# thnak/image_super_resolution

Measured on AMD Instinct MI355X. Metric: 4x SR megapixels/sec (HR output) + PSNR vs reference CPU path, higher is better.
Workload: dtype fp16; 1 GPU; ResNet(16, 0.2, scaleRate=4) RRDB inference, 128x128->512x512; global_batch=16, per_gpu_batch=16, lr_size=128, scale=4, parallelism=dp1 (independent tile shards), streams_per_gpu=1, hip_graph=True, trunk=persistent chain kernel, storage=fp16 activations and packed weights, fp32 accumulation

## Files before the change

### image_super_resolution_amd/csrc/trunk.hip

```cpp
#include "trunk_common.h"

namespace isr {

size_t trunk_state_words(int n, int ha, int wa) {
    const size_t tiles = (size_t)n * (ha / tk::TH) * (wa / tk::TW);
    return trunk_rec_off((int)tiles) + 1024 * 16;
}

__global__ __launch_bounds__(1024) void trunk_prep_kernel(const isr_conv_desc* layers, const int32_t* kinds, int nl,
                                                          int n, int ha, int wa, unsigned* state, int th,
                                                          int h16) {
    extern __shared__ __attribute__((aligned(16))) char smem[];
    unsigned* err = reinterpret_cast<unsigned*>(smem);
    const int L = threadIdx.x;
    const int nbx = wa / tk::TW, nby = ha / th, ntiles = n * nbx * nby;
    const size_t ro = trunk_rec_off(ntiles);
    if (L == 0) *err = 0;
    __syncthreads();
    const isr_conv_desc& g0 = layers[0];
    if (L < nl) {
        const isr_conv_desc& d = layers[L];
        unsigned e = 0;
        auto same_geo = [&](const isr_view& v) {
            return v.hp == g0.x.hp && v.wp == g0.x.wp && v.cs == g0.x.cs && v.pad == g0.x.pad && v.coff % 16 == 0 &&
                   v.pad >= 1;
        };
        const int kind = kinds[L];
        const bool masked = kind == 2;
        if (d.n != n || d.ha != ha || d.wa != wa || d.h != g0.h || d.w != g0.w) e |= 1;
        if (!same_geo(d.x) || !same_geo(d.y) || (d.r2.data && !same_geo(d.r2)) || (masked && !same_geo(d.m))) e |= 2;
        if (kind == 0 || kind == 2 ? d.cout != 32 : (kind == 1 ? d.cout != 64 : true)) e |= 4;
        if (d.cin % 16 || d.cin < 64 || d.cin / 16 > 120 || !d.bias || ((uintptr_t)d.bias & 15)) e |= 8;
        if (d.f16 != h16 || d.shuffle != 1 || d.x_sub2 || d.taps || d.y2.data || (d.m.data != nullptr) != masked ||
            (masked && (d.m_c0 != 0 || d.slope != 1.f || d.r1.data || d.r2.data || d.s1 != 1.f || d.s2 != 1.f)))
            e |= 16;
        int fold = 0;
        uint16_t idv = 0;
        if (d.r1.data) {
            const float inv = 1.f / d.s1;
            float back;
            if (h16) {
                const _Float16 hi = (_Float16)inv;
                idv = __builtin_bit_cast(uint16_t, hi);
                back = (float)hi;
            } else {
                const __bf16 bi = (__bf16)inv;
                idv = __builtin_bit_cast(uint16_t, bi);
                back = (float)bi;
            }
            const bool alias = d.r1.data == d.x.data && d.r1.coff == d.x.coff && d.r1_cn == 0;
            if (!alias || kind != 1 || d.slope != 1.f || back != inv) e |= 32;
            fold = 1;
        } else if (d.r2.data) {
            e |= 32;
        }
        int first_new = tk::NEED_NONE;
        if (L > 0) {
            const isr_conv_desc& p = layers[L - 1];
            const int lo = p.y.coff, hi = p.y.coff + p.cout;
            first_new = d.cin / 16;
            if (p.y.data == d.x.data) {
                for (int c = 0; c < d.cin / 16; ++c) {
                    const int c0 = d.x.coff + 16 * c;
                    if (c0 < hi && lo < c0 + 16) {
                        first_new = c;
                        break;
                    }
                }
            }
        }
        TrunkRec rec;
        rec.x = (uint64_t)(uintptr_t)d.x.data;
        rec.y = (uint64_t)(uintptr_t)d.y.data;
        rec.w = (uint64_t)(uintptr_t)d.wpack;
        rec.b = (uint64_t)(uintptr_t)d.bias;
        rec.r2 = (uint64_t)(uintptr_t)(masked ? d.m.data : d.r2.data);
        rec.planes = (uint32_t)(d.x.coff / 16) | (uint32_t)(d.y.coff / 16) << 16;
        rec.shape = (uint32_t)((masked ? d.m.coff : d.r2.coff) / 16) | (uint32_t)(d.cin / 16) << 16 |
                    (uint32_t)(kind & 255) << 24;
        rec.deps = (uint32_t)first_new | (uint32_t)fold << 8 | (uint32_t)idv << 16;
        rec.slope = masked ? d.mslope : d.slope;
        rec.s1 = d.s1;
        rec.s2 = d.s2;
        const uint32_t* src = reinterpret_cast<const uint32_t*>(&rec);
        uint32_t* dst = state + ro + (size_t)L * 16;
#pragma unroll
        for (int i = 0; i < 16; ++i) dst[i] = src[i];
        if (e) atomicOr(err, e);
    }
    __syncthreads();
    if (L == 0) {
        const size_t plane = (size_t)g0.x.hp * g0.x.wp * 32;
        const unsigned e = *err | (plane >= 0x7fffffffull ? 64u : 0u) | (nl > 1024 ? 128u : 0u);
        uint32_t* geo = state + ro - 16;
        const int32_t gv[16] = {n, g0.h, g0.w, ha, wa, g0.x.hp, g0.x.wp, g0.x.cs / 16, g0.x.pad, nbx, nby, ntiles,
                                (int32_t)e, 0, 0, 0};
#pragma unroll
        for (int i = 0; i < 16; ++i) geo[i] = (uint32_t)gv[i];
        state[0] = state[0] + 1u;
    }
}

int trunk_prep_launch(const isr_chain_desc* cd, int th, hipStream_t s) {
    hipLaunchKernelGGL(trunk_prep_kernel, dim3(1), dim3(1024), 16, s, cd->layers, cd->kinds, cd->nl, cd->n, cd->ha,
                       cd->wa, cd->state, th, cd->f16 ? 1 : 0);
    return hipGetLastError() == hipSuccess ? 0 : -1;
}

#ifdef ISR_TUNING
__device__ unsigned long long* g_trunk_stamps;
#endif
__device__ __forceinline__ void trunk_stamp(int L, int t, int ntiles, int slot) {
#ifdef ISR_TUNING
    unsigned long long* p = g_trunk_stamps;
    if (p != nullptr && threadIdx.x == 0 && L >= 75 && L < 90) {
        unsigned long long v;
        asm volatile("s_memrealtime %0\n\ts_waitcnt lgkmcnt(0)" : "=s"(v)::"memory");
        p[((size_t)(L - 75) * ntiles + t) * 8 + slot] = v;
    }
#else
    (void)L, (void)t, (void)ntiles, (void)slot;
#endif
}

#if ISR_TRUNK_MFMA16_PROBE
__device__ __forceinline__ f32x16 mfma32_probe16(bf16x8 a, bf16x8 b, f32x16 acc) {
    f32x4 c0 = __builtin_shufflevector(acc, acc, 0, 1, 2, 3), c1 = __builtin_shufflevector(acc, acc, 4, 5, 6, 7);
    c0 = __builtin_amdgcn_mfma_f32_16x16x32_bf16(a, b, c0, 0, 0, 0);
    c1 = __builtin_amdgcn_mfma_f32_16x16x32_bf16(a, b, c1, 0, 0, 0);
    f32x4 c2 = __builtin_shufflevector(acc, acc, 8, 9, 10, 11), c3 = __builtin_shufflevector(acc, acc, 12, 13, 14, 15);
    f32x8 lo = __builtin_shufflevector(c0, c1, 0, 1, 2, 3, 4, 5, 6, 7), hi = __builtin_shufflevector(c2, c3, 0, 1, 2, 3, 4, 5, 6, 7);
    return __builtin_shufflevector(lo, hi, 0, 1, 2, 3, 4, 5, 6, 7, 8, 9, 10, 11, 12, 13, 14, 15);
}
#endif

#ifdef ISR_TUNING
__device__ int g_trunk_knobs[4];
static int g_trunk_per_cu = 0;
__device__ __forceinline__ int trunk_abl_load() { return __builtin_amdgcn_readfirstlane(g_trunk_knobs[0]); }
#else
__device__ __forceinline__ int trunk_abl_load() { return 0; }
#endif

#ifdef ISR_TUNING
__device__ unsigned long long* g_item_stamps;
#endif
__device__ __forceinline__ void item_stamp(int L, int first_tile, int ch, int slot, int wm) {
#ifdef ISR_TUNING
    unsigned long long* p = g_item_stamps;
    const int w = wave_id();
    if (p != nullptr && first_tile && (threadIdx.x & 63) == 0 && (w == 0 || w == wm / 2) && (L == 77 || L == 79)) {
        const unsigned long long v = __builtin_amdgcn_s_memtime();
        p[((((size_t)blockIdx.x * 2 + (L == 79)) * 16 + ch) * 2 + (w != 0)) * 8 + slot] = v;
    }
#else
    (void)L, (void)first_tile, (void)ch, (void)slot, (void)wm;
#endif
}

struct TrunkArgs {
    unsigned* state;
    int rec_off;
    int nl;
    int acquire;
};


__device__ __forceinline__ void glds4(const void* gsrc, void* lds) {
    __builtin_amdgcn_global_load_lds(gsrc, ISR_LDS_PTR(lds), 4, 0, 0);
}

template <int WM_, int R_, int NST_, int TH_ = 16, int XM_ = 0, int NTP_ = 0>
struct TK {
    static constexpr int WM = WM_, R = R_, NST = NST_;
    static constexpr int HALO_AUX = 16 | ((NTP_ & 1) ? 2 : 0), STORE_AUX = 16 | ((NTP_ & 2) ? 2 : 0);
    static constexpr int XM = XM_;
    static constexpr int NT = 64 * WM;
    static constexpr int TH = TH_;
    static constexpr int HQ = (TH + 2) * tk::HC;
    static constexpr int HP = (HQ + 31) / 32;
    static_assert(R * WM == TH, "the waves cover the tile rows");
    static_assert(NST >= 2 && NST <= 4, "ring depth");
    static constexpr int HPW = (HP + WM - 1) / WM;
    static constexpr int WPW = (tk::WPF + WM - 1) / WM;
    static constexpr int SLOT = (HP + tk::WPF) * 1024;
    static constexpr int BIAS_OFF = NST * SLOT;
    static constexpr int LDS = BIAS_OFF + 4 * 256;
    static_assert(LDS <= 163840, "LDS budget");
    static constexpr int BPC = 163840 / LDS < 2 ? 163840 / LDS : 2;
    static constexpr int WPS = BPC * WM / 4;
    static constexpr int NSET = WPS >= 4 ? 1 : 2;
};

struct Src {
    const char* x;
    uint32_t h0;
    const char* w;
    const float* b;
    int wpc;
    uint32_t xbytes, wbytes;
};

template <class K>
struct TrunkCtx {
    static constexpr int TH = K::TH;
    unsigned* state;
    unsigned gen;
    int acquire;
    int hp, wp, cs16, pad, h, w, nbx, nby, ntiles;
    uint32_t pstride;
    uint32_t hoff[K::HPW];
    int abl;
};

template <class C>
__device__ __forceinline__ Src src_of(const C& c, const_rec& rec, int t) {
    const int bx = t % c.nbx, tmp = t / c.nbx, by = tmp % c.nby, img = tmp / c.nby;
    Src s;
    s.x = (const char*)(uintptr_t)rec.x + (size_t)((uint32_t)img * c.cs16 + rec_xp(rec)) * c.pstride;
    s.h0 = (uint32_t)(((by * C::TH - 1 + c.pad) * c.wp + (bx * tk::TW - 1 + c.pad)) * 32);
    s.w = (const char*)(uintptr_t)rec.w;
    s.b = (const float*)(uintptr_t)rec.b;
    s.wpc = rec_kind(rec) == 1 ? tk::WPF : tk::WPG;
    s.xbytes = c.pstride;
    s.wbytes = (uint32_t)(rec_nch(rec) * s.wpc * 1024);
    return s;
}

template <int WM, int HPW, int WPW, int SLOTB, int BIASB, int HP, int HAUX = 16>
__device__ __forceinline__ uint32_t stage_chunk_k(const uint32_t* hoff, uint32_t pstride, int abl, const Src& s,
                                                  int chunk, int slot, bool with_bias, int bslot) {
    extern __shared__ __attribute__((aligned(16))) char smem[];
    const int wave = wave_id(), lane = threadIdx.x & 63;
    char* dst = smem + slot * SLOTB;
    uint32_t n = 0;
    const auto rx = rsrc_n(s.x + (size_t)chunk * pstride, s.xbytes);
    const uint32_t so = s.h0;
    if (!(abl & 1)) {
#pragma unroll
        for (int k = 0; k < HPW; ++k) {
            const int j = wave + WM * k;
            if (j < HP) {
                __builtin_amdgcn_raw_ptr_buffer_load_lds(rx, ISR_LDS_PTR(dst + j * 1024), 16, hoff[k], so, 0, HAUX);
                ++n;
            }
        }
    }
    const auto rw = rsrc_n(s.w, s.wbytes);
    const uint32_t wo = (uint32_t)(chunk * s.wpc * 1024);
    char* wd = dst + HP * 1024;
#pragma unroll
    for (int k = 0; k < WPW; ++k) {
        const int j = wave + WM * k;
        if (j < s.wpc && !(abl & 8)) {
            __builtin_amdgcn_raw_ptr_buffer_load_lds(rw, ISR_LDS_PTR(wd + j * 1024), 16, lane * 16, wo + j * 1024, 0, 0);
            ++n;
        }
    }
    if (with_bias && wave == 0) {
        if (lane < (s.wpc == tk::WPG ? 32 : 64))
            __builtin_amdgcn_raw_ptr_buffer_load_lds(rsrc_n(s.b, s.wpc == tk::WPG ? 128u : 256u), ISR_LDS_PTR(smem + BIASB + bslot * 256), 4,
                                                     lane * 4, 0, 0, 0);
        ++n;
    }
    return n;
}

template <class K>
__device__ __forceinline__ uint32_t stage_chunk(const TrunkCtx<K>& c, const Src& s, int chunk, int slot, bool with_bias,
                                                int bslot) {
#ifdef ISR_TUNING
    if (chunk < 0 || (uint32_t)(chunk * s.wpc * 1024) >= s.wbytes || slot < 0 || slot >= K::NST ||
        bslot < 0 || bslot > 3) {
        if (threadIdx.x == 0) {
            __hip_atomic_store(c.state + 1, c.gen, __ATOMIC_RELAXED, __HIP_MEMORY_SCOPE_AGENT);
            __hip_atomic_fetch_add(c.state + 2, 1u, __ATOMIC_RELAXED, __HIP_MEMORY_SCOPE_AGENT);
        }
        return 0;
    }
#endif
    if constexpr (K::NSET == 1) {
        int ln = threadIdx.x & 63;
        asm volatile("" : "+v"(ln));
        uint32_t ho[K::HPW];
#pragma unroll
        for (int k = 0; k < K::HPW; ++k) ho[k] = halo_piece_off<K::HQ>(wave_id() + K::WM * k, ln, c.wp);
        return stage_chunk_k<K::WM, K::HPW, K::WPW, K::SLOT, K::BIAS_OFF, K::HP, K::HALO_AUX>(ho, c.pstride, c.abl, s, chunk, slot,
                                                                          with_bias, bslot);
    }
    return stage_chunk_k<K::WM, K::HPW, K::WPW, K::SLOT, K::BIAS_OFF, K::HP, K::HALO_AUX>(c.hoff, c.pstride, c.abl, s, chunk, slot,
                                                                      with_bias, bslot);
}

#ifndef ISR_TRUNK_PRIO
#define ISR_TRUNK_PRIO 1
#endif
#ifndef ISR_TRUNK_REFILL_FIRST
#define ISR_TRUNK_REFILL_FIRST 0
#endif
constexpr bool kRefillFirst = ISR_TRUNK_REFILL_FIRST != 0;
#ifndef ISR_TRUNK_INTERLEAVE
#define ISR_TRUNK_INTERLEAVE 0
#endif
constexpr bool kTrunkInterleave = ISR_TRUNK_INTERLEAVE != 0;
constexpr int kTrunkInterleaveStep = ISR_TRUNK_INTERLEAVE == 2 ? 2 : 0;

struct Refill {
    bool on;
    Src src;
    const char* xb;
    uint32_t so, wo;
    char* dst;
    bool bias;
    int bslot;
};

template <int WM, int HPW, int WPW, int BIASB, int HP>
__device__ __forceinline__ uint32_t refill_piece_k(const uint32_t* hoff, int abl, const Refill& rf, const int p) {
    extern __shared__ __attribute__((aligned(16))) char smem[];
    const int wave = wave_id(), lane = threadIdx.x & 63;
    if (p < HPW) {
        const int j = wave + WM * p;
        if (!(abl & 1) && j < HP) {
            __builtin_amdgcn_raw_ptr_buffer_load_lds(rsrc_n(rf.xb, rf.src.xbytes), ISR_LDS_PTR(rf.dst + j * 1024), 16, hoff[p],
                                                     rf.so, 0, 16);
            return 1;
        }
        return 0;
    }
    if (p < HPW + WPW) {
        const int j = wave + WM * (p - HPW);
        if (j < rf.src.wpc) {
            __builtin_amdgcn_raw_ptr_buffer_load_lds(rsrc_n(rf.src.w, rf.src.wbytes), ISR_LDS_PTR(rf.dst + (HP + j) * 1024), 16,
                                                     lane * 16, rf.wo + j * 1024, 0, 0);
            return 1;
        }
        return 0;
    }
    if (p == HPW + WPW && rf.bias && wave == 0) {
        if (lane < (rf.src.wpc == tk::WPG ? 32 : 64))
            __builtin_amdgcn_raw_ptr_buffer_load_lds(rsrc_n(rf.src.b, rf.src.wpc == tk::WPG ? 128u : 256u), ISR_LDS_PTR(smem + BIASB + rf.bslot * 256), 4,
                                                     lane * 4, 0, 0, 0);
        return 1;
    }
    return 0;
}

template <class K>
__device__ __forceinline__ uint32_t refill_piece(const TrunkCtx<K>& c, const Refill& rf, const int p) {
    return refill_piece_k<K::WM, K::HPW, K::WPW, K::BIAS_OFF, K::HP>(c.hoff, c.abl, rf, p);
}

template <class K>
__device__ __forceinline__ Refill make_refill(const TrunkCtx<K>& c, const Src& s, int chunk, int slot, bool with_bias,
                                              int bslot) {
    extern __shared__ __attribute__((aligned(16))) char smem[];
    Refill rf;
    rf.on = true;
    rf.src = s;
    rf.xb = s.x + (size_t)chunk * c.pstride;
    rf.so = s.h0;
    rf.wo = (uint32_t)(chunk * s.wpc * 1024);
    rf.dst = smem + slot * K::SLOT;
    rf.bias = with_bias;
    rf.bslot = bslot;
#ifdef ISR_TUNING
    if (chunk < 0 || rf.wo >= s.wbytes || slot < 0 || slot >= K::NST || bslot < 0 || bslot > 3) {
        if (threadIdx.x == 0) {
            __hip_atomic_store(c.state + 1, c.gen, __ATOMIC_RELAXED, __HIP_MEMORY_SCOPE_AGENT);
            __hip_atomic_fetch_add(c.state + 2, 1u, __ATOMIC_RELAXED, __HIP_MEMORY_SCOPE_AGENT);
        }
        rf.on = false;
    }
#endif
    return rf;
}

struct Next {
    bool exists;
    int L, t;
    Src src;
    int first_new;
    int nch;
    bool self_dep;
};

template <class K>
struct Stream {
    int item;
    int staged;
    int tseq;
    uint32_t issued;
    uint32_t m0, m1, m2, m3;
    int pend_t;
    unsigned pend_v;
    uint32_t pend_mark;
    bool dep_next;
};

template <class K>
__device__ __forceinline__ void push_mark(Stream<K>& st) {
    const int pos = st.staged - st.item;
    const uint32_t v = st.issued;
    st.m0 = pos == 0 ? v : st.m0;
    st.m1 = pos == 1 ? v : st.m1;
    st.m2 = pos == 2 ? v : st.m2;
    st.m3 = pos >= 3 ? v : st.m3;
}

template <class K>
__device__ __forceinline__ void pop_mark(Stream<K>& st) {
    st.m0 = st.m1;
    st.m1 = st.m2;
    st.m2 = st.m3;
}

template <class K>
__device__ __forceinline__ void force_publish(const TrunkCtx<K>& c, Stream<K>& st) {
    if (st.pend_t < 0) return;
    asm volatile("s_waitcnt vmcnt(0)" ::: "memory");
    raw_barrier();
    if (threadIdx.x == 0)
        __hip_atomic_store(c.state + 4 + st.pend_t, st.pend_v, __ATOMIC_RELAXED, __HIP_MEMORY_SCOPE_AGENT);
    st.pend_t = -1;
}

template <class K, int NF, bool MASKED = false, bool H = false>
__device__ __forceinline__ void run_tile(const TrunkCtx<K>& c, Stream<K>& st, const_rec& rec, int L, int t,
                                         const Next& nx) {
    extern __shared__ __attribute__((aligned(16))) char smem[];
    constexpr int R = K::R, NST = K::NST, CT = 32 * NF, TN = 3, NA = R + 2;
    const int wave = wave_id(), lane = threadIdx.x & 63, l31 = lane & 31, hh = lane >> 5;
    const int bx = t % c.nbx, tmp = t / c.nbx, by = tmp % c.nby, img = tmp / c.nby;
    const int x0 = bx * tk::TW, y0 = by * K::TH;
    const int nch = rec_nch(rec);
    const int first_new = rec_first_new(rec);
    const unsigned need = c.gen * 1024u + (unsigned)L;
    const bool fold = NF == 2 && rec_fold(rec);
    const bool has_r2 = NF == 2 && rec.r2 != 0;
    constexpr bool masked = NF == 1 && MASKED;
    const Src me = src_of(c, rec, t);
    bool dep_ok = first_new == tk::NEED_NONE || st.dep_next;
    st.dep_next = false;
    const int bslot = st.tseq & 3;
    const int first_item = st.item;
    trunk_stamp(L, t, c.ntiles, 0);

    const uint32_t a_w = (uint32_t)(K::HP * 1024 + (2 * l31 + (hh ^ ((l31 >> 3) & 1))) * 16);
    uint32_t a_h[3];
#pragma unroll
    for (int dx = 0; dx < 3; ++dx)
        a_h[dx] = (uint32_t)((wave * R * tk::HC + l31 + dx) * 32 + 16 * (hh ^ (((l31 + dx) >> 3) & 1)));

    auto wait_deps = [&](int tt, unsigned nd) {
        force_publish(c, st);
        trunk_stamp(L, t, c.ntiles, 4);
        if (!(c.abl & 16)) dep_wait(c.state, nb_of(tt, c.nbx, c.nby), nd, c.gen);
        if (c.acquire) acquire_fence();
        trunk_stamp(L, t, c.ntiles, 5);
    };

    f32x16 acc[R][NF];

    const uint32_t idv = rec_idv(rec);
    auto do_chunk = [&](const int ch, auto fc_tag) {
        constexpr int FC = decltype(fc_tag)::value;
            const int slot = st.item % NST;
            const bool stamp_tile = t == (int)blockIdx.x;
            item_stamp(L, stamp_tile, ch, 0, K::WM);
            if (st.staged < st.item) {
                force_publish(c, st);
                if (ch >= first_new && !dep_ok) {
                    wait_deps(t, need);
                    dep_ok = true;
                }
                st.issued += stage_chunk(c, me, ch, slot, ch == 0, bslot);
                st.staged = st.item;
                push_mark(st);
            }
            wait_vm(st.issued - st.m0);
            item_stamp(L, stamp_tile, ch, 1, K::WM);
            raw_barrier();
            item_stamp(L, stamp_tile, ch, 2, K::WM);
            if (st.pend_t >= 0 && (int)(st.m0 - st.pend_mark) >= 0) {
                if (threadIdx.x == 0)
                    __hip_atomic_store(c.state + 4 + st.pend_t, st.pend_v, __ATOMIC_RELAXED, __HIP_MEMORY_SCOPE_AGENT);
                st.pend_t = -1;
            }
            if (ch == 0) {
                trunk_stamp(L, t, c.ntiles, 1);
                const float* bs = reinterpret_cast<const float*>(smem + K::BIAS_OFF + bslot * 256);
    #pragma unroll
                for (int f = 0; f < NF; ++f) {
                    f32x16 b0;
    #pragma unroll
                    for (int j = 0; j < 4; ++j) {
                        const f32x4 q = *reinterpret_cast<const f32x4*>(bs + f * 32 + 8 * j + 4 * hh);
    #pragma unroll
                        for (int e = 0; e < 4; ++e) b0[4 * j + e] = q[e];
                    }
    #pragma unroll
                    for (int r = 0; r < R; ++r) acc[r][f] = b0;
                }
            }
            const char* sb = smem + slot * K::SLOT;
            constexpr int NSET = K::NSET;
            uint32_t aw = a_w, ah[3] = {a_h[0], a_h[1], a_h[2]};
            if constexpr (NSET == 1) {
                int ln = threadIdx.x & 63;
                asm volatile("" : "+v"(ln));
                const int q31 = ln & 31, qh = ln >> 5;
                aw = (uint32_t)(K::HP * 1024 + (2 * q31 + (qh ^ ((q31 >> 3) & 1))) * 16);
    #pragma unroll
                for (int dx = 0; dx < 3; ++dx)
                    ah[dx] = (uint32_t)((wave * R * tk::HC + q31 + dx) * 32 + 16 * (qh ^ (((q31 + dx) >> 3) & 1)));
            }
            bf16x8 fb[NSET][TN][NF], fa[NSET][NA];
            auto read_one = [&](int dx, int idx, int set) {
                if (idx < TN * NF) {
                    const int dyi = idx / NF, f = idx % NF;
                    fb[set][dyi][f] = lds_read16(sb + aw + ((dyi * 3 + dx) * CT * 2 + f * 64) * 16);
                } else {
                    const int ia = idx - TN * NF;
                    fa[set][ia] = lds_read16(sb + ah[dx] + ia * tk::HC * 32);
                }
            };
            auto read_fb = [&](int dx, int dyi, int set) {
    #pragma unroll
                for (int f = 0; f < NF; ++f) read_one(dx, dyi * NF + f, set);
            };
            auto read_step0 = [&]() {
                if constexpr (K::NSET == 1) {
                    read_fb(0, 0, 0);
    #pragma unroll
                    for (int ia = 0; ia < R; ++ia) read_one(0, TN * NF + ia, 0);
                    __builtin_amdgcn_sched_barrier(0);
                    return;
                }
                read_fb(0, 0, 0);
    #pragma unroll
                for (int ia = 0; ia < R; ++ia) read_one(0, TN * NF + ia, 0);
                read_fb(0, 1, 0);
                read_one(0, TN * NF + R, 0);
                read_fb(0, 2, 0);
                read_one(0, TN * NF + R + 1, 0);
                __builtin_amdgcn_sched_barrier(0);
            };
            if constexpr (!kRefillFirst) read_step0();

            Refill rf;
            rf.on = false;
            while (st.staged < st.item + NST - 1) {
                const int off = st.staged + 1 - first_item;
                const int nslot = (st.staged + 1) % NST;
                if (off < nch) {
                    if (off >= first_new && !dep_ok) {
                        wait_deps(t, need);
                        dep_ok = true;
                    }
                    if constexpr (kTrunkInterleave && NST == 2) {
                        if (st.staged + 1 == st.item + NST - 1) {
                            rf = make_refill(c, me, off, nslot, false, 0);
                            ++st.staged;
                            break;
                        }
                    }
                    st.issued += stage_chunk(c, me, off, nslot, false, 0);
                } else {
                    const int nc = off - nch;
                    if (!nx.exists || nc >= nx.nch) break;
                    if (nx.L > 0 && nc >= nx.first_new && !st.dep_next) {
                        if (nx.self_dep) break;
                        wait_deps(nx.t, c.gen * 1024u + (unsigned)nx.L);
                        st.dep_next = true;
                    }
                    if constexpr (kTrunkInterleave && NST == 2) {
                        if (st.staged + 1 == st.item + NST - 1) {
                            rf = make_refill(c, nx.src, nc, nslot, nc == 0, (bslot + 1) & 3);
                            ++st.staged;
                            break;
                        }
                    }
                    st.issued += stage_chunk(c, nx.src, nc, nslot, nc == 0, (bslot + 1) & 3);
                }
                ++st.staged;
                push_mark(st);
            }
            __builtin_amdgcn_sched_barrier(0);
            if constexpr (kRefillFirst) read_step0();
            item_stamp(L, stamp_tile, ch, 3, K::WM);
            uint32_t rf_n = 0;
#if ISR_TRUNK_PRIO == 1
            __builtin_amdgcn_s_setprio(1);
#endif

    #pragma unroll
            for (int stp = 0; stp < 3; ++stp) {
                const int cur = NSET == 2 ? (stp & 1) : 0;
                if constexpr (NSET == 1) {
                    if (stp > 0) {
                        read_fb(stp, 0, 0);
    #pragma unroll
                        for (int ia = 0; ia < R; ++ia) read_one(stp, TN * NF + ia, 0);
                        __builtin_amdgcn_sched_barrier(0);
                    }
                }
    #pragma unroll
                for (int dyi = 0; dyi < TN; ++dyi) {
                    if constexpr (NSET == 1) {
                        if (dyi + 1 < TN) {
                            read_fb(stp, dyi + 1, 0);
                            read_one(stp, TN * NF + dyi + R, 0);
                            __builtin_amdgcn_sched_barrier(0);
                        }
                    }
    #pragma unroll
                    for (int r = 0; r < R; ++r) {
#if ISR_TRUNK_MFMA16_PROBE
                        if constexpr (NF == 1) {
                            acc[r][0] = mfma32_probe16(fb[cur][dyi][0], fa[cur][r + dyi], acc[r][0]);
                        } else
#endif
    #pragma unroll
                        for (int f = 0; f < NF; ++f) acc[r][f] = mfma32t<H>(fb[cur][dyi][f], fa[cur][r + dyi], acc[r][f]);
                        if constexpr (NF == 2 && FC >= 0) {
                            if (dyi == 1 && stp == 1) {
                                const bf16x8 a = fold_a_bits<K::NSET == 1>(idv, FC & 1);
                                acc[r][FC >> 1] = mfma32t<H>(a, fa[cur][r + 1], acc[r][FC >> 1]);
                            }
                        }
                        if (NSET == 2 && stp + 1 < 3 && (dyi == 2 || r == 0))
                            read_one(stp + 1, TN * NF + r + dyi, cur ^ 1);
                        if (stp == kTrunkInterleaveStep && rf.on) rf_n += refill_piece<K>(c, rf, dyi * R + r);
                        __builtin_amdgcn_sched_barrier(0);
                    }
                    if (NSET == 2 && stp + 1 < 3) {
                        read_fb(stp + 1, dyi, cur ^ 1);
                        __builtin_amdgcn_sched_barrier(0);
                    }
                }
                if (stp == kTrunkInterleaveStep && rf.on) {
    #pragma unroll
                    for (int q = TN * R; q <= K::HPW + K::WPW; ++q) rf_n += refill_piece<K>(c, rf, q);
                    st.issued += rf_n;
                    push_mark(st);
                    __builtin_amdgcn_sched_barrier(0);
                }
            }
#if ISR_TRUNK_PRIO == 1
            __builtin_amdgcn_s_setprio(0);
#endif
            item_stamp(L, stamp_tile, ch, 4, K::WM);
            pop_mark(st);
    };
    int ch0 = 0;
    if constexpr (NF == 2) {
        if (fold && nch >= 4) {
            do_chunk(0, TIC<0>{});
            ++st.item;
            do_chunk(1, TIC<1>{});
            ++st.item;
            do_chunk(2, TIC<2>{});
            ++st.item;
            do_chunk(3, TIC<3>{});
            ++st.item;
            ch0 = 4;
        }
    }
    for (int ch = ch0; ch < nch; ++ch, ++st.item) do_chunk(ch, TIC<-1>{});
    trunk_stamp(L, t, c.ntiles, 2);

    if (!dep_ok && first_new != tk::NEED_NONE) wait_deps(t, need);

    {
        typedef __attribute__((ext_vector_type(4))) unsigned u32x4;
        const int xx = x0 + l31;
        const float slope = rec.slope, s1 = rec.s1, s2 = rec.s2;
        const bool scale2 = s2 != 1.f;
        const char* ybase = (const char*)(uintptr_t)rec.y + (size_t)((uint32_t)img * c.cs16 + rec_yp(rec)) * c.pstride;
        bf16x8 q2[R][NF][2];
        const char* r2base = (const char*)(uintptr_t)rec.r2 + (size_t)((uint32_t)img * c.cs16 + rec_r2p(rec)) * c.pstride;
        auto load_r2 = [&](int r) {
            const uint32_t pix = (uint32_t)((y0 + wave * R + r + c.pad) * c.wp + xx + c.pad);
#pragma unroll
            for (int f = 0; f < NF; ++f)
#pragma unroll
                for (int blk = 0; blk < 2; ++blk) {
                    const auto rr = rsrc_n(r2base + (size_t)(2 * f + blk) * c.pstride, c.pstride);
                    q2[r][f][blk] = __builtin_bit_cast(
                        bf16x8, __builtin_amdgcn_raw_buffer_load_b128(rr, pix * 32 + 16 * hh, 0, 16));
                }
            st.issued += NF * 2;
        };
        if (has_r2 || masked) load_r2(0);
#pragma unroll
        for (int r = 0; r < R; ++r) {
            if ((has_r2 || masked) && r + 1 < R) load_r2(r + 1);
            const int yy = y0 + wave * R + r;
            const bool valid = yy < c.h && xx < c.w;
            const uint32_t pix = (uint32_t)((yy + c.pad) * c.wp + xx + c.pad);
#pragma unroll
            for (int f = 0; f < NF; ++f) {
                float v[16];
#pragma unroll
                for (int g = 0; g < 16; ++g) v[g] = acc[r][f][g];
#pragma unroll
                for (int k = 0; k < 4; ++k) {
                    swap_halves(v[k], v[4 + k]);
                    swap_halves(v[8 + k], v[12 + k]);
                }
#pragma unroll
                for (int blk = 0; blk < 2; ++blk) {
                    float* u = v + 8 * blk;
#pragma unroll
                    for (int e = 0; e < 8; ++e) {
                        if (masked)
                            u[e] = elt<H>(q2[r][f][blk], e) > 0.f ? u[e] : u[e] * slope;
                        else
                            u[e] = u[e] >= 0.f ? u[e] : u[e] * slope;
                        if (fold) u[e] = u[e] * s1;
                        if (has_r2) {
                            u[e] = u[e] * s2 + elt<H>(q2[r][f][blk], e);
                        } else {
                            if (scale2) u[e] *= s2;
                        }
                        if (!valid) u[e] = 0.f;
                    }
                    const auto yr = rsrc_n(ybase + (size_t)(2 * f + blk) * c.pstride, c.pstride);
                    const uint32_t off = pix * 32 + 16 * hh;
                    const bf16x8 tq = pack8<H>(u);
                    if (!(c.abl & 4)) {
                        __builtin_amdgcn_raw_buffer_store_b128(__builtin_bit_cast(u32x4, tq), yr, off, 0, K::STORE_AUX);
                        ++st.issued;
                    }
                }
            }
        }
    }
    trunk_stamp(L, t, c.ntiles, 3);
    st.pend_t = t;
    st.pend_v = c.gen * 1024u + (unsigned)(L + 1);
    st.pend_mark = st.issued;
    ++st.tseq;
}

template <class K, bool H = false>
__global__ __launch_bounds__(K::NT, K::WPS) void trunk_kernel(TrunkArgs a) {
    TrunkCtx<K> c;
    c.state = a.state;
    c.acquire = a.acquire;
    c.gen = __hip_atomic_load(a.state, __ATOMIC_RELAXED, __HIP_MEMORY_SCOPE_AGENT);
    const_geo& g = *(const_geo*)(uintptr_t)(a.state + a.rec_off - 16);
    const_rec* recs = (const_rec*)(uintptr_t)(a.state + a.rec_off);
    if (g.err != 0) {
        if (threadIdx.x == 0) {
            __hip_atomic_store(a.state + 1, c.gen, __ATOMIC_RELAXED, __HIP_MEMORY_SCOPE_AGENT);
            __hip_atomic_fetch_add(a.state + 2, 1u, __ATOMIC_RELAXED, __HIP_MEMORY_SCOPE_AGENT);
        }
        return;
    }
    c.hp = g.hp;
    c.wp = g.wp;
    c.cs16 = g.cs16;
    c.pad = g.pad;
    c.h = g.h;
    c.w = g.w;
    c.nbx = g.nbx;
    c.nby = g.nby;
    c.ntiles = g.ntiles;
    c.pstride = (uint32_t)(c.hp * c.wp * 32);
    c.abl = trunk_abl_load();
    {
        const int wave = wave_id(), lane = threadIdx.x & 63;
#pragma unroll
        for (int k = 0; k < K::HPW; ++k) c.hoff[k] = K::NSET == 1 ? 0u : halo_piece_off<K::HQ>(wave + K::WM * k, lane, c.wp);
    }
    const int G = gridDim.x, b = K::XM ? xcd_remap((int)blockIdx.x, (int)gridDim.x) : (int)blockIdx.x;
#if ISR_TRUNK_PRIO == 2
    if (__builtin_amdgcn_readfirstlane(b) >= G / 2) __builtin_amdgcn_s_setprio(1);
#endif
    Stream<K> st;
    st.item = 0;
    st.staged = 0;
    st.tseq = 0;
    st.issued = 0;
    st.m0 = st.m1 = st.m2 = st.m3 = 0;
    st.pend_t = -1;
    st.pend_v = 0;
    st.pend_mark = 0;
    st.dep_next = false;
    if (b < c.ntiles) {
        st.issued += stage_chunk(c, src_of(c, recs[0], b), 0, 0, true, 0);
        st.m0 = st.issued;
        for (int L = 0; L < a.nl; ++L) {
            const_rec& rec = recs[L];
            for (int t = b; t < c.ntiles; t += G) {
                Next nx;
                nx.exists = true;
                if (t + G < c.ntiles) {
                    nx.L = L;
                    nx.t = t + G;
                } else if (L + 1 < a.nl) {
                    nx.L = L + 1;
                    nx.t = b;
                } else {
                    nx.exists = false;
                    nx.L = L;
                    nx.t = t;
                }
                const_rec& nrec = recs[nx.L];
                nx.src = src_of(c, nrec, nx.t);
                nx.first_new = rec_first_new(nrec);
                nx.nch = rec_nch(nrec);
                {
                    const int bx = t % c.nbx, tq = t / c.nbx, by = tq % c.nby, im = tq / c.nby;
                    const int bx2 = nx.t % c.nbx, nq = nx.t / c.nbx, by2 = nq % c.nby, im2 = nq / c.nby;
                    nx.self_dep = im == im2 && abs(bx - bx2) <= 1 && abs(by - by2) <= 1;
                }
                const int kind = rec_kind(rec);
                if (kind == 0) run_tile<K, 1, false, H>(c, st, rec, L, t, nx);
                else if (kind == 2) run_tile<K, 1, true, H>(c, st, rec, L, t, nx);
                else run_tile<K, 2, false, H>(c, st, rec, L, t, nx);
            }
        }
    }
    asm volatile("s_waitcnt vmcnt(0)" ::: "memory");
    __syncthreads();
    if (threadIdx.x == 0 && st.pend_t >= 0)
        __hip_atomic_store(c.state + 4 + st.pend_t, st.pend_v, __ATOMIC_RELAXED, __HIP_MEMORY_SCOPE_AGENT);
}

template <class K, bool H = false>
static int trunk_launch_k(const isr_chain_desc* cd, hipStream_t s) {
    if (cd->ha % K::TH || cd->wa % tk::TW || cd->nl < 1 || cd->nl > 1024) return -2;
    const int nbx = cd->wa / tk::TW, nby = cd->ha / K::TH;
    const long long ntiles = (long long)cd->n * nbx * nby;
    if (ntiles <= 0 || ntiles > (1 << 24)) return -2;
    static thread_local int cached_dev = -1, cached_per_cu = 0, cached_cus = 0;
    int dev = 0;
    if (hipGetDevice(&dev) != hipSuccess) return -1;
    const void* kern = (const void*)trunk_kernel<K, H>;
    if (dev != cached_dev) {
        (void)hipFuncSetAttribute(kern, hipFuncAttributeMaxDynamicSharedMemorySize, K::LDS);
        int per_cu = 0;
        if (hipOccupancyMaxActiveBlocksPerMultiprocessor(&per_cu, kern, K::NT, K::LDS) != hipSuccess) return -1;
        int cus = 0;
        if (hipDeviceGetAttribute(&cus, hipDeviceAttributeMultiprocessorCount, dev) != hipSuccess || cus <= 0) return -1;
        cached_dev = dev;
        cached_per_cu = per_cu < K::BPC ? per_cu : K::BPC;
        cached_cus = cus;
    }
    int per_cu = cached_per_cu;
#ifdef ISR_TUNING
    if (g_trunk_per_cu > 0 && g_trunk_per_cu < per_cu) per_cu = g_trunk_per_cu;
#endif
    if (per_cu < 1) return -4;
    const long long slots = (long long)per_cu * cached_cus;
    const int grid = (int)(ntiles < slots ? ntiles : slots);
    const int rec_off = (int)trunk_rec_off((int)ntiles);
    trunk_prep_launch(cd, K::TH, s);
    TrunkArgs a;
    a.state = cd->state;
    a.rec_off = rec_off;
    a.nl = cd->nl;
    a.acquire = cd->acquire;
    hipLaunchKernelGGL((trunk_kernel<K, H>), dim3(grid), dim3(K::NT), K::LDS, s, a);
    return hipGetLastError() == hipSuccess ? 0 : -1;
}

#ifndef ISR_TRUNK_XCD
#define ISR_TRUNK_XCD 0
#endif
using TK_PAIR = TK<4, 4, 2, 16, ISR_TRUNK_XCD>;

#ifdef ISR_TUNING
using TK_DEEP = TK<8, 2, 4>;
using TK_T32 = TK<8, 4, 2, 32>;
using TK_QUAD = TK<8, 2, 2>;
using TK_PAIR_X = TK<4, 4, 2, 16, 1>;
using TK_PAIR_NTH = TK<4, 4, 2, 16, 0, 1>;
using TK_PAIR_NTS = TK<4, 4, 2, 16, 0, 2>;
#endif

int trunk_launch(const isr_chain_desc* cd, hipStream_t s, int form) {
    if (cd->f16) return form == 0 ? trunk_launch_k<TK_PAIR, true>(cd, s) : -3;
    if (form == 0) return trunk_launch_k<TK_PAIR>(cd, s);
#ifdef ISR_TUNING
    if (form == 2) return trunk_launch_k<TK_T32>(cd, s);
    if (form == 4) return trunk_launch_k<TK_QUAD>(cd, s);
    if (form == 5) return trunk_launch_k<TK_PAIR_X>(cd, s);
    if (form == 6) return trunk_launch_k<TK_PAIR_NTH>(cd, s);
    if (form == 7) return trunk_launch_k<TK_PAIR_NTS>(cd, s);
    if (form == 1) return trunk_launch_k<TK_DEEP>(cd, s);
#endif
    return -3;
}

#ifdef ISR_TUNING
int trunk_knobs_set(const int* k) {
    g_trunk_per_cu = k[1];
    return hipMemcpyToSymbol(HIP_SYMBOL(g_trunk_knobs), k, 4 * sizeof(int)) == hipSuccess ? 0 : -1;
}
int trunk_stamps_set(void* p) { return hipMemcpyToSymbol(HIP_SYMBOL(g_trunk_stamps), &p, sizeof(p)) == hipSuccess ? 0 : -1; }
int trunk_item_stamps_set(void* p) {
    return hipMemcpyToSymbol(HIP_SYMBOL(g_item_stamps), &p, sizeof(p)) == hipSuccess ? 0 : -1;
}
#else
int trunk_knobs_set(const int*) { return -2; }
int trunk_stamps_set(void*) { return -2; }
int trunk_item_stamps_set(void*) { return -2; }
#endif

}
```

### image_super_resolution_amd/csrc/trunk_common.h

```cpp
#pragma once
#include "isr_common.h"

namespace isr {

namespace tk {
constexpr int TH = 16;
constexpr int TW = 32;
constexpr int HR = TH + 2, HC = TW + 2, HQ = HR * HC;
constexpr int HP = (HQ + 31) / 32;
constexpr int WPG = 9, WPF = 18;
constexpr int NEED_NONE = 255;
}

struct TrunkRec {
    uint64_t x, y, w, b, r2;
    uint32_t planes;
    uint32_t shape;
    uint32_t deps;
    float slope, s1, s2;
};
static_assert(sizeof(TrunkRec) == 64, "record size");

struct TrunkGeo {
    int32_t n, h, w, ha, wa, hp, wp, cs16, pad, nbx, nby, ntiles, err, r0, r1, r2;
};

static inline __host__ __device__ size_t trunk_rec_off(int ntiles) {
    return ((size_t)ntiles + 4 + 15) / 16 * 16 + 16;
}

size_t trunk_state_words(int n, int ha, int wa);

typedef const __attribute__((address_space(4))) TrunkRec const_rec;
typedef const __attribute__((address_space(4))) TrunkRec const_rec_t;
typedef const __attribute__((address_space(4))) TrunkGeo const_geo;
__device__ __forceinline__ int rec_xp(const_rec_t& r) { return (int)(r.planes & 0xffff); }
__device__ __forceinline__ int rec_yp(const_rec_t& r) { return (int)(r.planes >> 16); }
__device__ __forceinline__ int rec_r2p(const_rec_t& r) { return (int)(r.shape & 0xffff); }
__device__ __forceinline__ int rec_nch(const_rec_t& r) { return (int)((r.shape >> 16) & 255); }
__device__ __forceinline__ int rec_kind(const_rec_t& r) { return (int)(r.shape >> 24); }
__device__ __forceinline__ int rec_first_new(const_rec_t& r) { return (int)(r.deps & 255); }
__device__ __forceinline__ bool rec_fold(const_rec_t& r) { return ((r.deps >> 8) & 1) != 0; }
__device__ __forceinline__ uint32_t rec_idv(const_rec_t& r) { return r.deps >> 16; }

__device__ __forceinline__ void raw_barrier() {
    asm volatile("s_waitcnt lgkmcnt(0)" ::: "memory");
    __builtin_amdgcn_s_barrier();
}

__device__ __forceinline__ int nb_of(int t, int nbx, int nby) {
    const int lane = threadIdx.x & 63;
    if (lane >= 9) return -1;
    const int bx = t % nbx, tmp = t / nbx, by = tmp % nby, img = tmp / nby;
    const int yy = by + lane / 3 - 1, xx = bx + lane % 3 - 1;
    return (yy >= 0 && yy < nby && xx >= 0 && xx < nbx) ? (img * nby + yy) * nbx + xx : -1;
}

#ifndef ISR_TRUNK_SPIN_SLEEP
#define ISR_TRUNK_SPIN_SLEEP 1
#endif

__device__ __forceinline__ unsigned poll_load(const unsigned* progress, int nb) {
    return __hip_atomic_load(progress + (nb < 0 ? 0 : nb), __ATOMIC_RELAXED, __HIP_MEMORY_SCOPE_AGENT);
}

__device__ __forceinline__ void dep_wait(unsigned* state, int nb, unsigned need, unsigned gen) {
    const unsigned* progress = state + 4;
    for (unsigned spins = 0;; ++spins) {
        const unsigned v = poll_load(progress, nb);
        if (__all(nb < 0 || (int)(v - need) >= 0)) break;
        if ((spins & 255) == 255 && __hip_atomic_load(state + 1, __ATOMIC_RELAXED, __HIP_MEMORY_SCOPE_AGENT) == gen)
            break;
        if (spins > (1u << 18)) {
            if ((threadIdx.x & 63) == 0) {
                __hip_atomic_store(state + 1, gen, __ATOMIC_RELAXED, __HIP_MEMORY_SCOPE_AGENT);
                __hip_atomic_fetch_add(state + 2, 1u, __ATOMIC_RELAXED, __HIP_MEMORY_SCOPE_AGENT);
            }
            break;
        }
        __builtin_amdgcn_s_sleep(ISR_TRUNK_SPIN_SLEEP);
    }
}

__device__ __forceinline__ void acquire_fence() {
    if ((threadIdx.x & 63) == 0) __builtin_amdgcn_fence(__ATOMIC_ACQUIRE, "agent");
    asm volatile("s_waitcnt vmcnt(0)" ::: "memory");
}

__device__ __forceinline__ __amdgpu_buffer_rsrc_t rsrc_n(const void* p, uint32_t bytes) {
    return __builtin_amdgcn_make_buffer_rsrc(const_cast<void*>(p), (short)0, (int)bytes, 0x00020000);
}

template <int HQ>
__device__ __forceinline__ uint32_t halo_piece_off(int j, int lane, int wp) {
    const int u = j * 64 + lane;
    const int q = u >> 1;
    if (q >= HQ) return 0;
    const int row = q / tk::HC, col = q - row * tk::HC;
    const int cc = (u & 1) ^ ((col >> 3) & 1);
    return (uint32_t)((row * wp + col) * 32 + cc * 16);
}

__device__ __forceinline__ void wait_vm(uint32_t n) {
#define ISR_VMW(k)                                        \
    case k:                                               \
        asm volatile("s_waitcnt vmcnt(" #k ")" ::: "memory"); \
        break;
    switch (n) {
        ISR_VMW(1) ISR_VMW(2) ISR_VMW(3) ISR_VMW(4) ISR_VMW(5) ISR_VMW(6) ISR_VMW(7) ISR_VMW(8) ISR_VMW(9)
        ISR_VMW(10) ISR_VMW(11) ISR_VMW(12) ISR_VMW(13) ISR_VMW(14) ISR_VMW(15) ISR_VMW(16) ISR_VMW(17)
        ISR_VMW(18) ISR_VMW(19) ISR_VMW(20) ISR_VMW(21) ISR_VMW(22) ISR_VMW(23) ISR_VMW(24) ISR_VMW(25)
        ISR_VMW(26) ISR_VMW(27) ISR_VMW(28) ISR_VMW(29) ISR_VMW(30) ISR_VMW(31) ISR_VMW(32) ISR_VMW(33)
        ISR_VMW(34) ISR_VMW(35) ISR_VMW(36) ISR_VMW(37) ISR_VMW(38) ISR_VMW(39) ISR_VMW(40) ISR_VMW(41)
        ISR_VMW(42) ISR_VMW(43) ISR_VMW(44) ISR_VMW(45) ISR_VMW(46) ISR_VMW(47) ISR_VMW(48) ISR_VMW(49)
        ISR_VMW(50) ISR_VMW(51) ISR_VMW(52) ISR_VMW(53) ISR_VMW(54) ISR_VMW(55) ISR_VMW(56) ISR_VMW(57)
        ISR_VMW(58) ISR_VMW(59) ISR_VMW(60) ISR_VMW(61) ISR_VMW(62) ISR_VMW(63)
        default: asm volatile("s_waitcnt vmcnt(0)" ::: "memory"); break;
    }
#undef ISR_VMW
}

template <int V> struct TIC { static constexpr int value = V; };

template <bool FRESH = false>
__device__ __forceinline__ bf16x8 fold_a_bits(uint32_t idv, int h16) {
    int lane = threadIdx.x & 63;
    if constexpr (FRESH) asm volatile("" : "+v"(lane));
    const int j = (lane & 31) - 16 * h16 - 8 * (lane >> 5);
    typedef __attribute__((ext_vector_type(4))) unsigned u32x4;
    u32x4 r;
#pragma unroll
    for (int d = 0; d < 4; ++d) r[d] = j == 2 * d ? idv : (j == 2 * d + 1 ? idv << 16 : 0u);
    return __builtin_bit_cast(bf16x8, r);
}


int trunk_prep_launch(const isr_chain_desc* cd, int th, hipStream_t s);

}
```

Baseline: 631.4 MPix/s.

## Specialize trunk chunk pipeline into compile-time roles with static ring slots

Replaces the generic per-chunk staging loop in the persistent trunk kernel with role-specialized chunk variants (first, second, steady, dep, loop, last). Each role issues a fixed double-buffer prefetch with compile-time LDS slot indices and simplified vmcnt waits. The last chunk prefetches the next tile's first chunk, and the Next descriptor is computed lazily. The aim is to cut per-chunk bookkeeping, the switch-based waitcnt and scalar overhead on the hot loop. The cost is larger code size and more template instantiations, plus a coarse waitcnt on the first chunk that may over-wait.

```diff
diff --git a/image_super_resolution_amd/csrc/trunk.hip b/image_super_resolution_amd/csrc/trunk.hip
--- a/image_super_resolution_amd/csrc/trunk.hip
+++ b/image_super_resolution_amd/csrc/trunk.hip
@@ -425,11 +425,50 @@
     st.pend_t = -1;
 }
 
+__device__ __forceinline__ bool next_item(int L, int t, int b, int G, int ntiles, int nl, int& nL, int& nt) {
+    nL = L;
+    nt = t;
+    if (t + G < ntiles) {
+        nt = t + G;
+        return true;
+    }
+    if (L + 1 < nl) {
+        nL = L + 1;
+        nt = b;
+        return true;
+    }
+    return false;
+}
+
+template <class C>
+__device__ __forceinline__ bool tiles_adjacent(const C& c, int t, int t2) {
+    const int bx = t % c.nbx, tq = t / c.nbx, by = tq % c.nby, im = tq / c.nby;
+    const int bx2 = t2 % c.nbx, nq = t2 / c.nbx, by2 = nq % c.nby, im2 = nq / c.nby;
+    return im == im2 && abs(bx - bx2) <= 1 && abs(by - by2) <= 1;
+}
+
+template <class K>
+constexpr bool kChunkRoles = K::NST == 2 && K::NSET == 2 && !kTrunkInterleave;
+
+enum : int {
+    CR_GENERAL,
+    CR_FIRST,
+    CR_SECOND,
+    CR_STEADY,
+    CR_DEP,
+    CR_LOOP,
+    CR_LAST
+};
+
 template <class K, int NF, bool MASKED = false, bool H = false>
-__device__ __forceinline__ void run_tile(const TrunkCtx<K>& c, Stream<K>& st, const_rec& rec, int L, int t,
-                                         const Next& nx) {
+__device__ __forceinline__ void run_tile(const TrunkCtx<K>& c, Stream<K>& st, const_rec* recs, int L, int t,
+                                         int nxL, int nxt, bool nx_exists) {
     extern __shared__ __attribute__((aligned(16))) char smem[];
     constexpr int R = K::R, NST = K::NST, CT = 32 * NF, TN = 3, NA = R + 2;
+    constexpr bool ROLES = kChunkRoles<K> && !MASKED;
+    constexpr bool FULL = ROLES && NF == 1;
+    constexpr int WPC = NF == 2 ? tk::WPF : tk::WPG;
+    const_rec& rec = recs[L];
     const int wave = wave_id(), lane = threadIdx.x & 63, l31 = lane & 31, hh = lane >> 5;
     const int bx = t % c.nbx, tmp = t / c.nbx, by = tmp % c.nby, img = tmp / c.nby;
     const int x0 = bx * tk::TW, y0 = by * K::TH;
@@ -440,6 +479,19 @@
     const bool has_r2 = NF == 2 && rec.r2 != 0;
     constexpr bool masked = NF == 1 && MASKED;
     const Src me = src_of(c, rec, t);
+    Next nx;
+    if constexpr (!ROLES) {
+        const_rec& nrec = recs[nxL];
+        nx.exists = nx_exists;
+        nx.L = nxL;
+        nx.t = nxt;
+        nx.src = src_of(c, nrec, nxt);
+        nx.first_new = rec_first_new(nrec);
+        nx.nch = rec_nch(nrec);
+        nx.self_dep = tiles_adjacent(c, t, nxt);
+    }
+    const char* xn = me.x;
+    uint32_t wo = 0;
     bool dep_ok = first_new == tk::NEED_NONE || st.dep_next;
     st.dep_next = false;
     const int bslot = st.tseq & 3;
@@ -460,14 +512,74 @@
         trunk_stamp(L, t, c.ntiles, 5);
     };
 
+    auto stage_own = [&](const int sl) {
+        char* dst = smem + sl * K::SLOT;
+        uint32_t n = 0;
+        const auto rx = rsrc_n(xn, c.pstride);
+        if (!(c.abl & 1)) {
+#pragma unroll
+            for (int k = 0; k < K::HPW; ++k) {
+                const int j = wave + K::WM * k;
+                if (K::WM * k + K::WM <= K::HP || j < K::HP) {
+                    __builtin_amdgcn_raw_ptr_buffer_load_lds(rx, ISR_LDS_PTR(dst + j * 1024), 16, c.hoff[k], me.h0, 0,
+                                                             K::HALO_AUX);
+                    ++n;
+                }
+            }
+        }
+        if (!(c.abl & 8)) {
+            const auto rw = rsrc_n(me.w, me.wbytes);
+#pragma unroll
+            for (int k = 0; k < (WPC + K::WM - 1) / K::WM; ++k) {
+                const int j = wave + K::WM * k;
+                if (K::WM * k + K::WM <= WPC || j < WPC) {
+                    __builtin_amdgcn_raw_ptr_buffer_load_lds(rw, ISR_LDS_PTR(dst + (K::HP + j) * 1024), 16, lane * 16,
+                                                             wo + j * 1024, 0, 0);
+                    ++n;
+                }
+            }
+        }
+        xn += c.pstride;
+        wo += WPC * 1024;
+        return n;
+    };
+
     f32x16 acc[R][NF];
 
     const uint32_t idv = rec_idv(rec);
-    auto do_chunk = [&](const int ch, auto fc_tag) {
-        constexpr int FC = decltype(fc_tag)::value;
-            const int slot = st.item % NST;
+    auto do_chunk = [&](const int ch, auto fc_tag, auto s_tag, auto role_tag) {
+        constexpr int FC = decltype(fc_tag)::value, S = decltype(s_tag)::value, ROLE = decltype(role_tag)::value;
+        static_assert((ROLE == CR_GENERAL) == !ROLES, "roles on the production ring only");
+            const int slot = S >= 0 ? S : st.item % NST;
             const bool stamp_tile = t == (int)blockIdx.x;
             item_stamp(L, stamp_tile, ch, 0, K::WM);
+            bool ring_ok = true;
+            if constexpr (ROLE == CR_FIRST) {
+                if (st.staged < st.item) {
+                    force_publish(c, st);
+                    if (first_new == 0 && !dep_ok) {
+                        wait_deps(t, need);
+                        dep_ok = true;
+                    }
+                    st.issued += stage_chunk(c, me, 0, slot, true, bslot);
+                    st.staged = st.item;
+                    st.m0 = st.issued;
+                }
+                xn += c.pstride;
+                wo += WPC * 1024;
+                wait_vm_coarse(st.issued - st.m0);
+            } else if constexpr (ROLE != CR_GENERAL) {
+#ifdef ISR_TUNING
+                if (st.issued != st.m0) {
+                    ring_ok = false;
+                    if (threadIdx.x == 0) {
+                        __hip_atomic_store(c.state + 1, c.gen, __ATOMIC_RELAXED, __HIP_MEMORY_SCOPE_AGENT);
+                        __hip_atomic_fetch_add(c.state + 2, 1u, __ATOMIC_RELAXED, __HIP_MEMORY_SCOPE_AGENT);
+                    }
+                }
+#endif
+                asm volatile("s_waitcnt vmcnt(0)" ::: "memory");
+            } else {
             if (st.staged < st.item) {
                 force_publish(c, st);
                 if (ch >= first_new && !dep_ok) {
@@ -479,15 +591,18 @@
                 push_mark(st);
             }
             wait_vm(st.issued - st.m0);
+            }
             item_stamp(L, stamp_tile, ch, 1, K::WM);
             raw_barrier();
             item_stamp(L, stamp_tile, ch, 2, K::WM);
+            if constexpr (ROLE == CR_GENERAL || ROLE == CR_FIRST || ROLE == CR_SECOND) {
             if (st.pend_t >= 0 && (int)(st.m0 - st.pend_mark) >= 0) {
                 if (threadIdx.x == 0)
                     __hip_atomic_store(c.state + 4 + st.pend_t, st.pend_v, __ATOMIC_RELAXED, __HIP_MEMORY_SCOPE_AGENT);
                 st.pend_t = -1;
             }
-            if (ch == 0) {
+            }
+            if (ROLE == CR_FIRST || (ROLE == CR_GENERAL && ch == 0)) {
                 trunk_stamp(L, t, c.ntiles, 1);
                 const float* bs = reinterpret_cast<const float*>(smem + K::BIAS_OFF + bslot * 256);
     #pragma unroll
@@ -550,6 +665,40 @@
 
             Refill rf;
             rf.on = false;
+            const bool last = ROLE == CR_LAST || (ROLE == CR_LOOP && ch == nch - 1);
+            if constexpr (ROLE == CR_LAST || ROLE == CR_LOOP) {
+                if (last && nx_exists && ring_ok) {
+                    const_rec& nrec = recs[nxL];
+                    bool go = true;
+                    if (nxL > 0 && rec_first_new(nrec) == 0) {
+                        if (tiles_adjacent(c, t, nxt)) {
+                            go = false;
+                        } else {
+                            wait_deps(nxt, c.gen * 1024u + (unsigned)nxL);
+                            st.dep_next = true;
+                        }
+                    }
+                    if (go) {
+                        st.issued += stage_chunk(c, src_of(c, nrec, nxt), 0, slot ^ 1, true, (bslot + 1) & 3);
+                        ++st.staged;
+                        st.m1 = st.issued;
+                    }
+                }
+            }
+            if constexpr (ROLE != CR_GENERAL && ROLE != CR_LAST) {
+                if constexpr (ROLE != CR_STEADY) {
+                    if (!last && ch + 1 >= first_new && !dep_ok) {
+                        wait_deps(t, need);
+                        dep_ok = true;
+                    }
+                }
+                if (!last && ring_ok) {
+                    st.issued += stage_own(slot ^ 1);
+                    ++st.staged;
+                    st.m1 = st.issued;
+                }
+            }
+            if constexpr (ROLE == CR_GENERAL)
             while (st.staged < st.item + NST - 1) {
                 const int off = st.staged + 1 - first_item;
                 const int nslot = (st.staged + 1) % NST;
@@ -652,22 +801,67 @@
 #endif
             item_stamp(L, stamp_tile, ch, 4, K::WM);
             pop_mark(st);
+            ++st.item;
     };
-    int ch0 = 0;
-    if constexpr (NF == 2) {
-        if (fold && nch >= 4) {
-            do_chunk(0, TIC<0>{});
-            ++st.item;
-            do_chunk(1, TIC<1>{});
-            ++st.item;
-            do_chunk(2, TIC<2>{});
-            ++st.item;
-            do_chunk(3, TIC<3>{});
-            ++st.item;
-            ch0 = 4;
-        }
-    }
-    for (int ch = ch0; ch < nch; ++ch, ++st.item) do_chunk(ch, TIC<-1>{});
+    if constexpr (ROLES) {
+        int ch = 0;
+        auto in_slot = [&](auto fc_tag, auto role_tag) {
+            if constexpr (!FULL) do_chunk(ch, fc_tag, TIC<-1>{}, role_tag);
+            else if (st.item & 1) do_chunk(ch, fc_tag, TIC<1>{}, role_tag);
+            else do_chunk(ch, fc_tag, TIC<0>{}, role_tag);
+            ++ch;
+        };
+        if constexpr (NF == 2) {
+            if (fold) {
+                in_slot(TIC<0>{}, TIC<CR_FIRST>{});
+                in_slot(TIC<1>{}, TIC<CR_SECOND>{});
+                in_slot(TIC<2>{}, TIC<CR_DEP>{});
+                in_slot(TIC<3>{}, TIC<CR_LOOP>{});
+            }
+        }
+        if (ch == 0) {
+            in_slot(TIC<-1>{}, TIC<CR_FIRST>{});
+            in_slot(TIC<-1>{}, TIC<CR_SECOND>{});
+        }
+        if (ch < nch) {
+            const int wb = first_new - 1;
+            int stop = wb >= ch && wb < nch - 1 ? wb : nch - 1;
+            if constexpr (!FULL) {
+                for (; ch < nch; ++ch) do_chunk(ch, TIC<-1>{}, TIC<-1>{}, TIC<CR_LOOP>{});
+            } else {
+                for (;;) {
+                    if (ch < stop && (st.item & 1)) {
+                        do_chunk(ch, TIC<-1>{}, TIC<1>{}, TIC<CR_STEADY>{});
+                        ++ch;
+                    }
+                    for (; ch + 1 < stop; ch += 2) {
+                        do_chunk(ch, TIC<-1>{}, TIC<0>{}, TIC<CR_STEADY>{});
+                        do_chunk(ch + 1, TIC<-1>{}, TIC<1>{}, TIC<CR_STEADY>{});
+                    }
+                    if (ch < stop) {
+                        do_chunk(ch, TIC<-1>{}, TIC<0>{}, TIC<CR_STEADY>{});
+                        ++ch;
+                    }
+                    if (ch >= nch - 1) break;
+                    in_slot(TIC<-1>{}, TIC<CR_DEP>{});
+                    stop = nch - 1;
+                }
+                in_slot(TIC<-1>{}, TIC<CR_LAST>{});
+            }
+        }
+    } else {
+        int ch0 = 0;
+        if constexpr (NF == 2) {
+            if (fold && nch >= 4) {
+                do_chunk(0, TIC<0>{}, TIC<-1>{}, TIC<CR_GENERAL>{});
+                do_chunk(1, TIC<1>{}, TIC<-1>{}, TIC<CR_GENERAL>{});
+                do_chunk(2, TIC<2>{}, TIC<-1>{}, TIC<CR_GENERAL>{});
+                do_chunk(3, TIC<3>{}, TIC<-1>{}, TIC<CR_GENERAL>{});
+                ch0 = 4;
+            }
+        }
+        for (int ch = ch0; ch < nch; ++ch) do_chunk(ch, TIC<-1>{}, TIC<-1>{}, TIC<CR_GENERAL>{});
+    }
     trunk_stamp(L, t, c.ntiles, 2);
 
     if (!dep_ok && first_new != tk::NEED_NONE) wait_deps(t, need);
@@ -795,32 +989,12 @@
         for (int L = 0; L < a.nl; ++L) {
             const_rec& rec = recs[L];
             for (int t = b; t < c.ntiles; t += G) {
-                Next nx;
-                nx.exists = true;
-                if (t + G < c.ntiles) {
-                    nx.L = L;
-                    nx.t = t + G;
-                } else if (L + 1 < a.nl) {
-                    nx.L = L + 1;
-                    nx.t = b;
-                } else {
-                    nx.exists = false;
-                    nx.L = L;
-                    nx.t = t;
-                }
-                const_rec& nrec = recs[nx.L];
-                nx.src = src_of(c, nrec, nx.t);
-                nx.first_new = rec_first_new(nrec);
-                nx.nch = rec_nch(nrec);
-                {
-                    const int bx = t % c.nbx, tq = t / c.nbx, by = tq % c.nby, im = tq / c.nby;
-                    const int bx2 = nx.t % c.nbx, nq = nx.t / c.nbx, by2 = nq % c.nby, im2 = nq / c.nby;
-                    nx.self_dep = im == im2 && abs(bx - bx2) <= 1 && abs(by - by2) <= 1;
-                }
+                int nxL, nxt;
+                const bool nx_exists = next_item(L, t, b, G, c.ntiles, a.nl, nxL, nxt);
                 const int kind = rec_kind(rec);
-                if (kind == 0) run_tile<K, 1, false, H>(c, st, rec, L, t, nx);
-                else if (kind == 2) run_tile<K, 1, true, H>(c, st, rec, L, t, nx);
-                else run_tile<K, 2, false, H>(c, st, rec, L, t, nx);
+                if (kind == 0) run_tile<K, 1, false, H>(c, st, recs, L, t, nxL, nxt, nx_exists);
+                else if (kind == 2) run_tile<K, 1, true, H>(c, st, recs, L, t, nxL, nxt, nx_exists);
+                else run_tile<K, 2, false, H>(c, st, recs, L, t, nxL, nxt, nx_exists);
             }
         }
     }
diff --git a/image_super_resolution_amd/csrc/trunk_common.h b/image_super_resolution_amd/csrc/trunk_common.h
--- a/image_super_resolution_amd/csrc/trunk_common.h
+++ b/image_super_resolution_amd/csrc/trunk_common.h
@@ -120,6 +120,12 @@
 #undef ISR_VMW
 }
 
+__device__ __forceinline__ void wait_vm_coarse(uint32_t n) {
+    if (n >= 16) asm volatile("s_waitcnt vmcnt(16)" ::: "memory");
+    else if (n >= 8) asm volatile("s_waitcnt vmcnt(8)" ::: "memory");
+    else asm volatile("s_waitcnt vmcnt(0)" ::: "memory");
+}
+
 template <int V> struct TIC { static constexpr int value = V; };
 
 template <bool FRESH = false>
```

Result: faster. 663.4 MPix/s, median of 6 (+5.1%).
